# Lemok00/IDEAS

Measured on AMD Instinct MI355X. Metric: train images/sec at 256x256 (G+D+Ex step), higher is better.
Workload: dtype f32; 1 GPU; IDEAS N=1 sigma=1 256x256 batch=32/GPU full G+D+Ex iteration (lazy R1 every 16, EMA), full-width nets, HIP kernels (BASELINE.json configs[2]); global_batch=32, parallelism=dp1, r1_steps_in_window=0, ranks=1

## Files before the change

ideas_amd/csrc/conv_b3_wgrad3.hip:

```cpp
#include "b3.hpp"
#include <type_traits>
#include <cstdlib>

namespace {

typedef short s16x4 __attribute__((ext_vector_type(4)));
typedef short s16x8 __attribute__((ext_vector_type(8)));

template <int S> struct W3 {
    static constexpr int XW = 15 * S + 3;
    static constexpr int NR = 4;
    static constexpr int XROWS = NR * XW;
    static constexpr int GROWS = 2 * 16;
    static constexpr int XPLANE = XROWS * 128, GPLANE = GROWS * 128;
    static constexpr int LDS = 3 * (XPLANE + GPLANE);
    static constexpr int XLOADS = (XW * 16 + 255) / 256;
};


template <int S, bool SCALE, bool REFLECT>
__global__ __launch_bounds__(256, 2) void conv_b3_wgrad3_kernel(float* __restrict__ gw, const float* __restrict__ gy,
                                                                const float* __restrict__ x, const float* __restrict__ in_scale,
                                                                const float* __restrict__ out_scale, ideas_conv_params p,
                                                                int tiles_ci, int tiles, int splits, int strips, int rows_per_split,
                                                                unsigned gy_bytes, unsigned x_bytes) {
    using L = W3<S>;
    constexpr int XW = L::XW, NR = L::NR;
    __shared__ __attribute__((aligned(16))) unsigned char smem[L::LDS];
    unsigned char* const sG = smem;
    unsigned char* const sX = smem + 3 * L::GPLANE;

    const int t = threadIdx.x, lane = t & 63, wave = t >> 6;
    int tile, split;
    splitk_xcd_map(blockIdx.x, tiles, splits, tile, split);
    const int o0 = (tile / tiles_ci) * 64, c0 = (tile % tiles_ci) * 64;
    const int strip = split % strips, range = split / strips;
    const int ox0 = strip * 16;
    const int rows_total = p.B * p.OH;
    const int R0 = range * rows_per_split;
    const int R1 = R0 + rows_per_split < rows_total ? R0 + rows_per_split : rows_total;
    if (R0 >= R1) return;

    const __amdgpu_buffer_rsrc_t rg = __builtin_amdgcn_make_buffer_rsrc((void*)gy, 0, (int)gy_bytes, (int)RSRC_FLAGS);
    const __amdgpu_buffer_rsrc_t rx = __builtin_amdgcn_make_buffer_rsrc((void*)x, 0, (int)x_bytes, (int)RSRC_FLAGS);
    const __amdgpu_buffer_rsrc_t rso = __builtin_amdgcn_make_buffer_rsrc((void*)out_scale, 0, SCALE ? p.B * p.Cout * 4 : 0, (int)RSRC_FLAGS);
    const __amdgpu_buffer_rsrc_t rsi = __builtin_amdgcn_make_buffer_rsrc((void*)in_scale, 0, SCALE ? p.B * p.Cin * 4 : 0, (int)RSRC_FLAGS);

    const int quad = t & 15, px = t >> 4;
    const unsigned g_cb = (unsigned)(o0 + quad * 4) * 4u, x_cb = (unsigned)(c0 + quad * 4) * 4u;
    auto xrow_of = [](int j) { return S == 1 ? j : (j & 1) * 17 + (j >> 1); };
    int x_lrow[L::XLOADS];
    bool x_on[L::XLOADS];
#pragma unroll
    for (int k = 0; k < L::XLOADS; ++k) {
        const int j = px + 16 * k;
        x_on[k] = j < XW;
        x_lrow[k] = xrow_of(j < XW ? j : 0);
    }

    struct Task { int b, wy, oy; bool mma, live; };
    int tk_b, tk_oa, tk_ob, tk_wy, tk_g;
    bool tk_done = false;
    {
        tk_g = R0;
        tk_b = R0 / p.OH;
        tk_oa = R0 - tk_b * p.OH;
        const int left = R1 - R0;
        tk_ob = tk_oa + left < p.OH ? tk_oa + left : p.OH;
        tk_wy = tk_oa * S;
    }
    auto next_task = [&]() -> Task {
        Task k;
        k.live = !tk_done;
        k.b = tk_b;
        k.wy = tk_wy;
        const int rel = tk_wy - tk_oa * S;
        k.mma = k.live && rel >= 2 && ((rel - 2) % S == 0);
        k.oy = tk_oa + (rel - 2) / S;
        if (!tk_done) {
            ++tk_wy;
            if (tk_wy > (tk_ob - 1) * S + 2) {
                tk_g += tk_ob - tk_oa;
                if (tk_g >= R1) tk_done = true;
                else {
                    ++tk_b;
                    tk_oa = 0;
                    tk_ob = R1 - tk_g < p.OH ? R1 - tk_g : p.OH;
                    tk_wy = 0;
                }
            }
        }
        return k;
    };

    struct Stage { float4 g, xv[L::XLOADS], sg, sx; };
    auto gload = [&](Stage& st, const Task& k) {
        int iy = k.wy + p.offy;
        bool yok = k.live;
        if (REFLECT) iy = reflect_coord(iy, p.IH);
        else yok = yok && (unsigned)iy < (unsigned)p.IH;
        const unsigned rowb = (unsigned)((k.b * p.IH + iy) * p.IW) * (unsigned)p.Cin * 4u + x_cb;
#pragma unroll
        for (int q = 0; q < L::XLOADS; ++q) {
            int ix = ox0 * S + p.offx + px + 16 * q;
            bool ok = yok && x_on[q];
            if (REFLECT) ix = reflect_coord(ix, p.IW);
            else ok = ok && (unsigned)ix < (unsigned)p.IW;
            st.xv[q] = buffer_load4(rx, ok ? rowb + (unsigned)ix * (unsigned)p.Cin * 4u : 0xffffffffu, 0);
        }
        const unsigned goff = (unsigned)(((k.b * p.OH + k.oy) * p.OW + ox0 + px) * p.Cout) * 4u + g_cb;
        st.g = buffer_load4(rg, k.mma ? goff : 0xffffffffu, 0);
        if (SCALE) {
            st.sg = buffer_load4(rso, (unsigned)(k.b * p.Cout) * 4u + g_cb, 0);
            st.sx = buffer_load4(rsi, (unsigned)(k.b * p.Cin) * 4u + x_cb, 0);
        }
    };
    auto put = [&](unsigned char* plane0, int plane_bytes, int row, float4 v, float4 sc) {
        if (SCALE) v = make_float4(mul_rn(v.x, sc.x), mul_rn(v.y, sc.y), mul_rn(v.z, sc.z), mul_rn(v.w, sc.w));
        const Split4 s = split4(v);
        unsigned char* a = plane0 + chunk_off(row, quad >> 1) + (quad & 1) * 8;
#pragma unroll
        for (int pl = 0; pl < 3; ++pl) *reinterpret_cast<uint2*>(a + pl * plane_bytes) = s.p[pl];
    };
    auto lstore = [&](const Stage& st, int n) {
        const int slot = n % NR;
#pragma unroll
        for (int q = 0; q < L::XLOADS; ++q)
            if (x_on[q]) put(sX, L::XPLANE, slot * XW + x_lrow[q], st.xv[q], st.sx);
        put(sG, L::GPLANE, (n & 1) * 16 + px, st.g, st.sg);
    };

    const int wo = wave >> 1, wc = wave & 1;
    const int li = lane & 31, lh = lane >> 5;
    const int g_q = lane & 15, g_row = g_q >> 2, g_piece = g_q & 3, g_cblk = (lane >> 4) & 1;
    auto lane_base = [&](unsigned region, int b, int cb) {
        const int r = b + 8 * lh + g_row;
        return region + (unsigned)(r * 128 + (((cb * 2 + (g_piece >> 1)) ^ ((((b + g_row) >> 1) & 1) << 2)) << 4) + (g_piece & 1) * 8);
    };
    const unsigned ldsG = (unsigned)(uintptr_t)(__attribute__((address_space(3))) unsigned char*)sG;
    const unsigned ldsX = (unsigned)(uintptr_t)(__attribute__((address_space(3))) unsigned char*)sX;
    unsigned baseG[4], baseX[4];
#pragma unroll
    for (int b = 0; b < 4; ++b) { baseG[b] = lane_base(ldsG, b, wo * 2 + g_cblk); baseX[b] = lane_base(ldsX, b, wc * 2 + g_cblk); }
    auto tr_ld = [&](unsigned addr) -> s16x4 {
        return __builtin_amdgcn_ds_read_tr16_b64_v4i16((__attribute__((address_space(3))) s16x4*)(uintptr_t)addr);
    };
    auto frag = [&](const unsigned (&base)[4], int plane_off, int r0) -> bf16x8 {
        const unsigned a0 = base[r0 & 3] + (unsigned)(plane_off + (r0 & ~3) * 128);
        const s16x4 a = tr_ld(a0);
        const s16x4 b = tr_ld(a0 + 512u);
        const s16x8 v = {a[0], a[1], a[2], a[3], b[0], b[1], b[2], b[3]};
        return __builtin_bit_cast(bf16x8, v);
    };

    f32x16 acc[9];
#pragma unroll
    for (int a = 0; a < 9; ++a)
#pragma unroll
        for (int r = 0; r < 16; ++r) acc[a][r] = 0.f;

    auto compute = [&](auto ph_) {
        constexpr int PH = decltype(ph_)::value;
        bf16x8 fa[3];
#pragma unroll
        for (int pl = 0; pl < 3; ++pl) fa[pl] = frag(baseG, pl * L::GPLANE, (PH & 1) * 16);
        auto loadB = [&](int tap, bf16x8 (&fb)[3]) {
            const int ty = tap / 3, tx = tap - 3 * ty;
            const int r0 = ((PH + 2 + ty) % NR) * XW + (S == 1 ? tx : (tx & 1) * 17 + (tx >> 1));
#pragma unroll
            for (int pl = 0; pl < 3; ++pl) fb[pl] = frag(baseX, pl * L::XPLANE, r0);
        };
        bf16x8 fb[5][2][3];
        loadB(0, fb[0][0]);
        loadB(1, fb[0][1]);
#pragma unroll
        for (int pr = 0; pr < 5; ++pr) {
            if (pr < 4) {
                loadB(2 * pr + 2, fb[pr + 1][0]);
                if (2 * pr + 3 < 9) loadB(2 * pr + 3, fb[pr + 1][1]);
            }
            __builtin_amdgcn_sched_barrier(0);
#pragma unroll
            for (int q = 0; q < 6; ++q) {
                acc[2 * pr] = __builtin_amdgcn_mfma_f32_32x32x16_bf16(fa[PA[q]], fb[pr][0][PB[q]], acc[2 * pr], 0, 0, 0);
                if (2 * pr + 1 < 9)
                    acc[2 * pr + 1] = __builtin_amdgcn_mfma_f32_32x32x16_bf16(fa[PA[q]], fb[pr][1][PB[q]], acc[2 * pr + 1], 0, 0, 0);
            }
            __builtin_amdgcn_sched_barrier(0);
        }
    };

    Stage st0, st1;
    Task k0 = next_task();
    gload(st0, k0);
    Task k1 = next_task();
    gload(st1, k1);
    lstore(st0, 0);
    __syncthreads();
    bool mma0 = k0.mma, mma1 = k1.mma, live0 = k0.live, live1 = k1.live;
    static_assert(NR == 4, "the step loop is unrolled over the ring positions");
    auto step = [&](auto ph_, Stage& ld, const Stage& stg) {
        constexpr int PH = decltype(ph_)::value;
        const Task k2 = next_task();
        gload(ld, k2);
        if (live1) lstore(stg, PH + 1);
        if (mma0) compute(ph_);
        __syncthreads();
        mma0 = mma1; live0 = live1; mma1 = k2.mma; live1 = k2.live;
    };
    while (live0) {
        step(std::integral_constant<int, 0>{}, st0, st1);
        if (!live0) break;
        step(std::integral_constant<int, 1>{}, st1, st0);
        if (!live0) break;
        step(std::integral_constant<int, 2>{}, st0, st1);
        if (!live0) break;
        step(std::integral_constant<int, 3>{}, st1, st0);
    }

    const int ci = c0 + wc * 32 + li;
#pragma unroll
    for (int tap = 0; tap < 9; ++tap)
#pragma unroll
        for (int r = 0; r < 16; ++r) {
            const int o = o0 + wo * 32 + (r & 3) + 8 * (r >> 2) + 4 * lh;
            atomicAdd(&gw[((int64_t)o * 9 + tap) * p.Cin + ci], acc[tap][r] * p.gain);
        }
}


template <int S>
int launch_wgrad3(float* gw, const void* gy, const void* x, const float* in_scale, const float* out_scale, const ideas_conv_params* p,
                  hipStream_t stream) {
    const int tiles_ci = p->Cin / 64, tiles = (p->Cout / 64) * tiles_ci;
    const int strips = p->OW / 16;
    const int64_t rows_total = (int64_t)p->B * p->OH;
    const int64_t slots = 512;
    int64_t spl = (4 * slots) / ((int64_t)tiles * strips);
    if (spl < 1 || rows_total / spl < 128) spl = (2 * slots) / ((int64_t)tiles * strips);
    if (spl < 1) spl = 1;
    const int64_t max_spl = rows_total / 16 > 0 ? rows_total / 16 : 1;
    if (spl > max_spl) spl = max_spl;
    int64_t per = ideas_cdiv(rows_total, spl);
    spl = ideas_cdiv(rows_total, per);
    const int64_t splits = spl * strips;
    if ((int64_t)tiles * splits > 0x7fffffffLL) return IDEAS_E_SHAPE;
    const unsigned gy_bytes = (unsigned)((int64_t)p->B * p->YH * p->YW * p->Cout * 4);
    const unsigned x_bytes = (unsigned)((int64_t)p->B * p->IH * p->IW * p->Cin * 4);
    auto go = [&](auto sc, auto rf) {
        hipLaunchKernelGGL((conv_b3_wgrad3_kernel<S, decltype(sc)::value, decltype(rf)::value>), dim3(splitk_grid(tiles, splits)),
                           dim3(256), 0, stream, gw, (const float*)gy, (const float*)x, in_scale, out_scale, *p, tiles_ci, tiles,
                           (int)splits, strips, (int)per, gy_bytes, x_bytes);
    };
    using T = std::true_type;
    using F = std::false_type;
    const bool sc = in_scale && out_scale;
    if (sc) { if (p->reflect) go(T{}, T{}); else go(T{}, F{}); }
    else { if (p->reflect) go(F{}, T{}); else go(F{}, F{}); }
    return ideas_launch_status();
}

}

bool ideas_b3_wgrad3_enabled() {
    const char* e = getenv("IDEAS_B3_WGRAD3");
    return !(e && e[0] == '0');
}

extern "C" int ideas_b3_wgrad3_supported(const ideas_conv_params* p) {
    if (!p) return 0;
    if (p->TY != 3 || p->TX != 3 || p->dy != 1 || p->dx != 1 || p->sy != p->sx || (p->sy != 1 && p->sy != 2)) return 0;
    if (p->osy != 1 || p->osx != 1 || p->ooy != 0 || p->oox != 0 || p->YH != p->OH || p->YW != p->OW) return 0;
    if (p->OW % 16 || p->Cin % 64 || p->Cout % 64) return 0;
    if (p->sy == 2) {
        const char* e = getenv("IDEAS_B3_WGRAD3_S2");
        if (e && e[0] == '0') return 0;
    }
    if (p->reflect && (p->IH < 2 || p->IW < 2)) return 0;
    if (p->offx > 0 || p->offx < -2 || p->offy > 0 || p->offy < -2) return 0;
    return (int64_t)p->B * p->IH * p->IW * p->Cin * 4 < 0xffffffffLL && (int64_t)p->B * p->YH * p->YW * p->Cout * 4 < 0xffffffffLL &&
           (int64_t)p->B * p->OH < 0x7fffffffLL;
}

int ideas_b3_wgrad3(float* gw, const void* gy, const void* x, const float* in_scale, const float* out_scale, const ideas_conv_params* p,
                    hipStream_t stream) {
    if (p->sy == 1) return launch_wgrad3<1>(gw, gy, x, in_scale, out_scale, p, stream);
    return launch_wgrad3<2>(gw, gy, x, in_scale, out_scale, p, stream);
}
```

Baseline: 82.63 images/sec.

## Add wide 128-output-channel wgrad3 kernel with 512 threads for large convolutions

Adds a second 3x3 weight-gradient kernel that covers 128 output channels per block with 8 waves. Each block shares the same input-x tile across two gradient images, which halves x loading and LDS staging per output channel. For stride 2 it uses a deeper row ring. A heuristic picks this kernel when the total work is large enough, and it also rescales split-K slot counts. The cost is lower occupancy (one block of 512 threads per CU, large LDS) and fewer blocks for split-K.

```diff
diff --git a/ideas_amd/csrc/conv_b3_wgrad3.hip b/ideas_amd/csrc/conv_b3_wgrad3.hip
--- a/ideas_amd/csrc/conv_b3_wgrad3.hip
+++ b/ideas_amd/csrc/conv_b3_wgrad3.hip
@@ -229,15 +229,267 @@
 }
 
 
+template <int S> struct W3W {
+    static constexpr int XW = 15 * S + 3;
+    static constexpr int NR = S == 1 ? 4 : 6;
+    static constexpr int UN = S == 1 ? 4 : 6;
+    static constexpr int XROWS = NR * XW;
+    static constexpr int GIMG = 2 * 16 * 128;
+    static constexpr int XPLANE = XROWS * 128, GPLANE = 2 * GIMG;
+    static constexpr int LDS = 3 * (XPLANE + GPLANE);
+    static constexpr int XLOADS = (S * XW + 31) / 32;
+};
+
+template <int S, bool SCALE, bool REFLECT>
+__global__ __launch_bounds__(512, 1) void conv_b3_wgrad3_wide_kernel(float* __restrict__ gw, const float* __restrict__ gy,
+                                                                     const float* __restrict__ x, const float* __restrict__ in_scale,
+                                                                     const float* __restrict__ out_scale, ideas_conv_params p,
+                                                                     int tiles_ci, int tiles, int splits, int strips,
+                                                                     int rows_per_split, unsigned gy_bytes, unsigned x_bytes) {
+    using L = W3W<S>;
+    constexpr int XW = L::XW, NR = L::NR, UN = L::UN;
+    __shared__ __attribute__((aligned(16))) unsigned char smem[L::LDS];
+    unsigned char* const sG = smem;
+    unsigned char* const sX = smem + 3 * L::GPLANE;
+
+    const int t = threadIdx.x, lane = t & 63, wave = t >> 6;
+    int tile, split;
+    splitk_xcd_map(blockIdx.x, tiles, splits, tile, split);
+    const int o0 = (tile / tiles_ci) * 128, c0 = (tile % tiles_ci) * 64;
+    const int strip = split % strips, range = split / strips;
+    const int ox0 = strip * 16;
+    const int rows_total = p.B * p.OH;
+    const int R0 = range * rows_per_split;
+    const int R1 = R0 + rows_per_split < rows_total ? R0 + rows_per_split : rows_total;
+    if (R0 >= R1) return;
+
+    const __amdgpu_buffer_rsrc_t rg = __builtin_amdgcn_make_buffer_rsrc((void*)gy, 0, (int)gy_bytes, (int)RSRC_FLAGS);
+    const __amdgpu_buffer_rsrc_t rx = __builtin_amdgcn_make_buffer_rsrc((void*)x, 0, (int)x_bytes, (int)RSRC_FLAGS);
+    const __amdgpu_buffer_rsrc_t rso = __builtin_amdgcn_make_buffer_rsrc((void*)out_scale, 0, SCALE ? p.B * p.Cout * 4 : 0, (int)RSRC_FLAGS);
+    const __amdgpu_buffer_rsrc_t rsi = __builtin_amdgcn_make_buffer_rsrc((void*)in_scale, 0, SCALE ? p.B * p.Cin * 4 : 0, (int)RSRC_FLAGS);
+
+    const int quad = t & 15, px = t >> 4, gpx = px & 15, gimg = t >> 8;
+    const unsigned g_cb = (unsigned)(o0 + gimg * 64 + quad * 4) * 4u, x_cb = (unsigned)(c0 + quad * 4) * 4u;
+    auto xrow_of = [](int j) { return S == 1 ? j : (j & 1) * 17 + (j >> 1); };
+    int x_lrow[L::XLOADS], x_col[L::XLOADS];
+    bool x_on[L::XLOADS], x_second[L::XLOADS];
+#pragma unroll
+    for (int k = 0; k < L::XLOADS; ++k) {
+        const int e = px + 32 * k;
+        x_on[k] = e < S * XW;
+        x_second[k] = e >= XW;
+        const int j = x_on[k] ? (e >= XW ? e - XW : e) : 0;
+        x_col[k] = j;
+        x_lrow[k] = xrow_of(j);
+    }
+
+    struct Task { int b, wy, oy; bool mma, live, first; };
+    int tk_b, tk_oa, tk_ob, tk_rel, tk_g;
+    bool tk_done = false;
+    {
+        tk_g = R0;
+        tk_b = R0 / p.OH;
+        tk_oa = R0 - tk_b * p.OH;
+        const int left = R1 - R0;
+        tk_ob = tk_oa + left < p.OH ? tk_oa + left : p.OH;
+        tk_rel = 0;
+    }
+    auto next_task = [&]() -> Task {
+        Task k;
+        k.live = !tk_done;
+        k.b = tk_b;
+        k.first = tk_rel == 0;
+        k.wy = S * (tk_oa + tk_rel) - (S - 1);
+        k.mma = k.live && tk_rel >= 3 - S;
+        k.oy = tk_oa + tk_rel - (3 - S);
+        if (!tk_done) {
+            ++tk_rel;
+            if (tk_rel > tk_ob - tk_oa - 1 + (3 - S)) {
+                tk_g += tk_ob - tk_oa;
+                if (tk_g >= R1) tk_done = true;
+                else {
+                    ++tk_b;
+                    tk_oa = 0;
+                    tk_ob = R1 - tk_g < p.OH ? R1 - tk_g : p.OH;
+                    tk_rel = 0;
+                }
+            }
+        }
+        return k;
+    };
+
+    float4 sc_g = make_float4(1.f, 1.f, 1.f, 1.f), sc_x = sc_g;
+    auto sload = [&](int b) {
+        if (SCALE) {
+            sc_g = buffer_load4(rso, (unsigned)(b * p.Cout) * 4u + g_cb, 0);
+            sc_x = buffer_load4(rsi, (unsigned)(b * p.Cin) * 4u + x_cb, 0);
+        }
+    };
+    struct Stage { float4 g, xv[L::XLOADS]; };
+    auto gload = [&](Stage& st, const Task& k) {
+        int iy0 = k.wy + p.offy, iy1 = iy0 + 1;
+        bool ok0 = k.live && !(S == 2 && k.first), ok1 = k.live;
+        if (REFLECT) { iy0 = reflect_coord(iy0, p.IH); iy1 = reflect_coord(iy1, p.IH); }
+        else { ok0 = ok0 && (unsigned)iy0 < (unsigned)p.IH; ok1 = ok1 && (unsigned)iy1 < (unsigned)p.IH; }
+        const unsigned rowb0 = (unsigned)((k.b * p.IH + (ok0 ? iy0 : 0)) * p.IW) * (unsigned)p.Cin * 4u + x_cb;
+        const unsigned rowb1 = (unsigned)((k.b * p.IH + (ok1 ? iy1 : 0)) * p.IW) * (unsigned)p.Cin * 4u + x_cb;
+#pragma unroll
+        for (int q = 0; q < L::XLOADS; ++q) {
+            const bool second = S == 2 && x_second[q];
+            int ix = ox0 * S + p.offx + x_col[q];
+            bool ok = x_on[q] && (second ? ok1 : ok0);
+            if (REFLECT) ix = reflect_coord(ix, p.IW);
+            else ok = ok && (unsigned)ix < (unsigned)p.IW;
+            st.xv[q] = buffer_load4(rx, ok ? (second ? rowb1 : rowb0) + (unsigned)ix * (unsigned)p.Cin * 4u : 0xffffffffu, 0);
+        }
+        const unsigned goff = (unsigned)(((k.b * p.OH + k.oy) * p.OW + ox0 + gpx) * p.Cout) * 4u + g_cb;
+        st.g = buffer_load4(rg, k.mma ? goff : 0xffffffffu, 0);
+    };
+    auto put = [&](unsigned char* plane0, int plane_bytes, int row, float4 v, float4 sc) {
+        if (SCALE) v = make_float4(mul_rn(v.x, sc.x), mul_rn(v.y, sc.y), mul_rn(v.z, sc.z), mul_rn(v.w, sc.w));
+        const Split4 s = split4(v);
+        unsigned char* a = plane0 + chunk_off(row, quad >> 1) + (quad & 1) * 8;
+#pragma unroll
+        for (int pl = 0; pl < 3; ++pl) *reinterpret_cast<uint2*>(a + pl * plane_bytes) = s.p[pl];
+    };
+    auto lstore = [&](const Stage& st, int n) {
+        const int slot0 = (S * n) % NR, slot1 = (S * n + S - 1) % NR;
+#pragma unroll
+        for (int q = 0; q < L::XLOADS; ++q)
+            if (x_on[q]) put(sX, L::XPLANE, ((S == 2 && x_second[q]) ? slot1 : slot0) * XW + x_lrow[q], st.xv[q], sc_x);
+        put(sG + gimg * L::GIMG, L::GPLANE, (n & 1) * 16 + gpx, st.g, sc_g);
+    };
+
+    const int wo = wave >> 1, wc = wave & 1;
+    const int lh = lane >> 5;
+    const int g_q = lane & 15, g_row = g_q >> 2, g_piece = g_q & 3, g_cblk = (lane >> 4) & 1;
+    auto lane_base = [&](unsigned region, int b, int cb) {
+        const int r = b + 8 * lh + g_row;
+        return region + (unsigned)(r * 128 + (((cb * 2 + (g_piece >> 1)) ^ ((((b + g_row) >> 1) & 1) << 2)) << 4) + (g_piece & 1) * 8);
+    };
+    const unsigned ldsG = (unsigned)(uintptr_t)(__attribute__((address_space(3))) unsigned char*)sG;
+    const unsigned ldsX = (unsigned)(uintptr_t)(__attribute__((address_space(3))) unsigned char*)sX;
+    unsigned baseX[4];
+#pragma unroll
+    for (int b = 0; b < 4; ++b) baseX[b] = lane_base(ldsX, b, wc * 2 + g_cblk);
+    const unsigned baseG = lane_base(ldsG + (unsigned)((wo >> 1) * L::GIMG), 0, (wo & 1) * 2 + g_cblk);
+    auto tr_ld = [&](unsigned addr) -> s16x4 {
+        return __builtin_amdgcn_ds_read_tr16_b64_v4i16((__attribute__((address_space(3))) s16x4*)(uintptr_t)addr);
+    };
+    auto frag_at = [&](unsigned a0) -> bf16x8 {
+        const s16x4 a = tr_ld(a0);
+        const s16x4 b = tr_ld(a0 + 512u);
+        const s16x8 v = {a[0], a[1], a[2], a[3], b[0], b[1], b[2], b[3]};
+        return __builtin_bit_cast(bf16x8, v);
+    };
+
+    f32x16 acc[9];
+#pragma unroll
+    for (int a = 0; a < 9; ++a)
+#pragma unroll
+        for (int r = 0; r < 16; ++r) acc[a][r] = 0.f;
+
+    auto compute = [&](auto ph_) {
+        constexpr int PH = decltype(ph_)::value;
+        bf16x8 fa[3];
+#pragma unroll
+        for (int pl = 0; pl < 3; ++pl) fa[pl] = frag_at(baseG + (unsigned)(pl * L::GPLANE + (PH & 1) * 16 * 128));
+        auto loadB = [&](int tap, bf16x8 (&fb)[3]) {
+            const int ty = tap / 3, tx = tap - 3 * ty;
+            const int r0 = ((S * PH + S - 3 + ty + NR) % NR) * XW + (S == 1 ? tx : (tx & 1) * 17 + (tx >> 1));
+#pragma unroll
+            for (int pl = 0; pl < 3; ++pl) fb[pl] = frag_at(baseX[r0 & 3] + (unsigned)(pl * L::XPLANE + (r0 & ~3) * 128));
+        };
+        bf16x8 fb[5][2][3];
+        loadB(0, fb[0][0]);
+        loadB(1, fb[0][1]);
+#pragma unroll
+        for (int pr = 0; pr < 5; ++pr) {
+            if (pr < 4) {
+                loadB(2 * pr + 2, fb[pr + 1][0]);
+                if (2 * pr + 3 < 9) loadB(2 * pr + 3, fb[pr + 1][1]);
+            }
+            __builtin_amdgcn_sched_barrier(0);
+#pragma unroll
+            for (int q = 0; q < 6; ++q) {
+                acc[2 * pr] = __builtin_amdgcn_mfma_f32_32x32x16_bf16(fa[PA[q]], fb[pr][0][PB[q]], acc[2 * pr], 0, 0, 0);
+                if (2 * pr + 1 < 9)
+                    acc[2 * pr + 1] = __builtin_amdgcn_mfma_f32_32x32x16_bf16(fa[PA[q]], fb[pr][1][PB[q]], acc[2 * pr + 1], 0, 0, 0);
+            }
+            __builtin_amdgcn_sched_barrier(0);
+        }
+    };
+
+    Stage st0, st1;
+    Task k0 = next_task();
+    gload(st0, k0);
+    Task k1 = next_task();
+    gload(st1, k1);
+    sload(k0.b);
+    lstore(st0, 0);
+    if (k1.live && k1.first) sload(k1.b);
+    __syncthreads();
+    bool mma0 = k0.mma, mma1 = k1.mma, live0 = k0.live, live1 = k1.live;
+    static_assert(UN % 2 == 0 && UN % (NR / S) == 0, "the step loop is unrolled over ring position x G buffer; the stage registers alternate");
+    auto step = [&](auto ph_, Stage& ld, const Stage& stg) {
+        constexpr int PH = decltype(ph_)::value;
+        const Task k2 = next_task();
+        gload(ld, k2);
+        if (live1) lstore(stg, (PH + 1) % UN);
+        if (k2.live && k2.first) sload(k2.b);
+        if (mma0) compute(ph_);
+        __syncthreads();
+        mma0 = mma1; live0 = live1; mma1 = k2.mma; live1 = k2.live;
+    };
+    while (live0) {
+        step(std::integral_constant<int, 0>{}, st0, st1);
+        if (!live0) break;
+        step(std::integral_constant<int, 1>{}, st1, st0);
+        if (!live0) break;
+        step(std::integral_constant<int, 2>{}, st0, st1);
+        if (!live0) break;
+        step(std::integral_constant<int, 3>{}, st1, st0);
+        if constexpr (UN == 6) {
+            if (!live0) break;
+            step(std::integral_constant<int, 4 % UN>{}, st0, st1);
+            if (!live0) break;
+            step(std::integral_constant<int, 5 % UN>{}, st1, st0);
+        }
+    }
+
+    int te = t;
+    asm volatile("" : "+v"(te));
+    const int e_wo = te >> 7, e_wc = (te >> 6) & 1, e_li = te & 31, e_lh = (te >> 5) & 1;
+    const int ci = c0 + e_wc * 32 + e_li;
+#pragma unroll
+    for (int tap = 0; tap < 9; ++tap)
+#pragma unroll
+        for (int r = 0; r < 16; ++r) {
+            const int o = o0 + e_wo * 32 + (r & 3) + 8 * (r >> 2) + 4 * e_lh;
+            atomicAdd(&gw[((int64_t)o * 9 + tap) * p.Cin + ci], acc[tap][r] * p.gain);
+        }
+}
+
+constexpr int64_t WGRAD3_WIDE_MIN_ROWS_S1 = 384, WGRAD3_WIDE_MIN_ROWS_S2 = 256, WGRAD3_WIDE_SLOTS = 256;
+bool wgrad3_choose(const ideas_conv_params* p) {
+    if (p->Cout % 128) return false;
+    const char* e = getenv("IDEAS_B3_WGRAD3_WIDE");
+    if (e && e[0]) return e[0] == '1' || (e[0] == '2' && p->sy == 2);
+    const int64_t steps = (int64_t)p->B * p->OH * (p->OW / 16) * (p->Cout / 128) * (p->Cin / 64);
+    return steps >= (p->sy == 1 ? WGRAD3_WIDE_MIN_ROWS_S1 : WGRAD3_WIDE_MIN_ROWS_S2) * WGRAD3_WIDE_SLOTS;
+}
+
 template <int S>
 int launch_wgrad3(float* gw, const void* gy, const void* x, const float* in_scale, const float* out_scale, const ideas_conv_params* p,
                   hipStream_t stream) {
-    const int tiles_ci = p->Cin / 64, tiles = (p->Cout / 64) * tiles_ci;
+    const bool wide = wgrad3_choose(p);
+    const int tiles_ci = p->Cin / 64, tiles = (p->Cout / (wide ? 128 : 64)) * tiles_ci;
     const int strips = p->OW / 16;
     const int64_t rows_total = (int64_t)p->B * p->OH;
-    const int64_t slots = 512;
-    int64_t spl = (4 * slots) / ((int64_t)tiles * strips);
-    if (spl < 1 || rows_total / spl < 128) spl = (2 * slots) / ((int64_t)tiles * strips);
+    const int64_t slots = wide ? WGRAD3_WIDE_SLOTS : 512;
+    const int waves = wide ? 2 : 4;
+    int64_t spl = (waves * slots) / ((int64_t)tiles * strips);
+    if (spl < 1 || rows_total / spl < 128) spl = (waves / 2 * slots) / ((int64_t)tiles * strips);
     if (spl < 1) spl = 1;
     const int64_t max_spl = rows_total / 16 > 0 ? rows_total / 16 : 1;
     if (spl > max_spl) spl = max_spl;
@@ -248,9 +500,14 @@
     const unsigned gy_bytes = (unsigned)((int64_t)p->B * p->YH * p->YW * p->Cout * 4);
     const unsigned x_bytes = (unsigned)((int64_t)p->B * p->IH * p->IW * p->Cin * 4);
     auto go = [&](auto sc, auto rf) {
-        hipLaunchKernelGGL((conv_b3_wgrad3_kernel<S, decltype(sc)::value, decltype(rf)::value>), dim3(splitk_grid(tiles, splits)),
-                           dim3(256), 0, stream, gw, (const float*)gy, (const float*)x, in_scale, out_scale, *p, tiles_ci, tiles,
-                           (int)splits, strips, (int)per, gy_bytes, x_bytes);
+        if (wide)
+            hipLaunchKernelGGL((conv_b3_wgrad3_wide_kernel<S, decltype(sc)::value, decltype(rf)::value>), dim3(splitk_grid(tiles, splits)),
+                               dim3(512), 0, stream, gw, (const float*)gy, (const float*)x, in_scale, out_scale, *p, tiles_ci, tiles,
+                               (int)splits, strips, (int)per, gy_bytes, x_bytes);
+        else
+            hipLaunchKernelGGL((conv_b3_wgrad3_kernel<S, decltype(sc)::value, decltype(rf)::value>), dim3(splitk_grid(tiles, splits)),
+                               dim3(256), 0, stream, gw, (const float*)gy, (const float*)x, in_scale, out_scale, *p, tiles_ci, tiles,
+                               (int)splits, strips, (int)per, gy_bytes, x_bytes);
     };
     using T = std::true_type;
     using F = std::false_type;
@@ -282,6 +539,10 @@
            (int64_t)p->B * p->OH < 0x7fffffffLL;
 }
 
+extern "C" int ideas_b3_wgrad3_wide(const ideas_conv_params* p) {
+    return ideas_b3_wgrad3_enabled() && ideas_b3_wgrad3_supported(p) && wgrad3_choose(p) ? 1 : 0;
+}
+
 int ideas_b3_wgrad3(float* gw, const void* gy, const void* x, const float* in_scale, const float* out_scale, const ideas_conv_params* p,
                     hipStream_t stream) {
     if (p->sy == 1) return launch_wgrad3<1>(gw, gy, x, in_scale, out_scale, p, stream);
```

Result: no change. 83.45 images/sec, median of 6 (+1.0%).
